# slobodaapl/nvit

Measured on AMD Instinct MI355X. Metric: images/sec (train step) nViT-B/16 224px, higher is better.
Workload: dtype bf16; 1 GPU; nViT-base 224px patches 8/16 T=784 C=768 L=12 H=12, full train step (fwd+bwd+clip+AdamW+renorm), synthetic images, formula weights; per_gpu_batch=128, global_batch=128, parallelism=dp1

## Files before the change

### nvit_amd/csrc/attn_mfma.hip

```cpp
#include <type_traits>

#include "common.h"

namespace {

constexpr int D = 64;
constexpr int ROWB = D * 2;
constexpr int TKV = 64;
constexpr int TILE_BYTES = TKV * ROWB;
constexpr float LOG2E = 1.4426950408889634f;

typedef __attribute__((address_space(3))) s16x4* lds_s16x4_ptr;

__device__ __forceinline__ float fast_exp2(float x) { return __builtin_amdgcn_exp2f(x); }

__device__ __forceinline__ int swz_off(int row, int chunk) { return row * ROWB + ((chunk ^ (row & 7)) << 4); }

__device__ __forceinline__ f32x4 mfma16(const uint4& a, const uint4& b, f32x4 c) {
  return __builtin_amdgcn_mfma_f32_16x16x32_bf16(__builtin_bit_cast(bf16x8, a), __builtin_bit_cast(bf16x8, b), c, 0, 0, 0);
}

__device__ __forceinline__ uint4 tr_frag(const char* tile, int row0, int col0, int l15, int lg) {
  const int q = l15 >> 2, p = l15 & 3;
  const int r0 = row0 + 4 * lg + q, r1 = r0 + 16;
// ... 21 lines not shown

__device__ __forceinline__ void store_tile32x64(const f32x4 (&g)[4][2], char* scr, bf16* dst, size_t ld, int nvalid,
                                                int lane) {
  const int l15 = lane & 15, lg = lane >> 4;
#pragma unroll
  for (int f = 0; f < 2; ++f)
#pragma unroll
    for (int df = 0; df < 4; ++df)
      *reinterpret_cast<uint2*>(scr + swz_off(16 * f + l15, 2 * df + (lg >> 1)) + 8 * (lg & 1)) = pack4(g[df][f]);
  __builtin_amdgcn_wave_barrier();
#pragma unroll
  for (int pass = 0; pass < 4; ++pass) {
    const int row = pass * 8 + (lane >> 3), chunk = lane & 7;
    const uint4 v = *reinterpret_cast<const uint4*>(scr + swz_off(row, chunk));
    if (row < nvalid) *reinterpret_cast<uint4*>(dst + (size_t)row * ld + chunk * 8) = v;
  }
}

__device__ __forceinline__ void glds16s(const void* sbase, unsigned voff, unsigned lds_off) {
  unsigned keep;
  const unsigned m = (unsigned)__builtin_amdgcn_readfirstlane((int)lds_off);
  const unsigned long long ub = (unsigned long long)(uintptr_t)sbase;
  const unsigned long long sb = (unsigned long long)(unsigned)__builtin_amdgcn_readfirstlane((int)(unsigned)ub) |
                                ((unsigned long long)(unsigned)__builtin_amdgcn_readfirstlane((int)(unsigned)(ub >> 32)) << 32);
  asm volatile(
      "s_mov_b32 %0, m0\n\ts_mov_b32 m0, %3\n\ts_nop 0\n\tglobal_load_lds_dwordx4 %1, %2\n\ts_mov_b32 m0, %0"
      : "=&s"(keep)
      : "v"(voff), "s"(sb), "s"(m)
      : "memory");
}
__device__ __forceinline__ void glds16s_pair(const void* sbase, unsigned voff0, unsigned voff1, unsigned lds_off) {
  unsigned keep;
  const unsigned m = (unsigned)__builtin_amdgcn_readfirstlane((int)lds_off);
  const unsigned long long ub = (unsigned long long)(uintptr_t)sbase;
  const unsigned long long sb = (unsigned long long)(unsigned)__builtin_amdgcn_readfirstlane((int)(unsigned)ub) |
                                ((unsigned long long)(unsigned)__builtin_amdgcn_readfirstlane((int)(unsigned)(ub >> 32)) << 32);
  asm volatile(
      "s_mov_b32 %0, m0\n\t"
      "s_mov_b32 m0, %4\n\ts_nop 0\n\tglobal_load_lds_dwordx4 %1, %3\n\t"
      "s_add_u32 m0, %4, 0x1000\n\ts_nop 0\n\tglobal_load_lds_dwordx4 %2, %3\n\t"
      "s_mov_b32 m0, %0"
      : "=&s"(keep)
      : "v"(voff0), "v"(voff1), "s"(sb), "s"(m)
      : "memory", "scc");
}
constexpr int TILE_DMA = 2;
__device__ __forceinline__ unsigned tile_voff(int i, unsigned ld_bytes, int lane, int wid) {
  const int r8 = lane >> 3, chunk = (lane & 7) ^ r8;
  return (unsigned)((i * 4 + wid) * 8 + r8) * ld_bytes + (unsigned)chunk * 16u;
}
__device__ __forceinline__ void tile_dma(const bf16* src, unsigned ld_bytes, int row_base, int nrows, unsigned tile_off,
                                         int lane, int wid, const unsigned (&voff)[TILE_DMA]) {
  const char* sb = reinterpret_cast<const char*>(src) + (size_t)row_base * ld_bytes;
  if (row_base + TKV <= nrows) {
    static_assert(TILE_DMA == 2, "glds16s_pair issues the tile's two pieces");
    glds16s_pair(sb, voff[0], voff[1], tile_off + wid * 1024);
  } else {
    const int r8 = lane >> 3, chunk = (lane & 7) ^ r8;
#pragma unroll
    for (int i = 0; i < TILE_DMA; ++i) {
      const int grp = i * 4 + wid;
      int row = grp * 8 + r8;
      row = row_base + row < nrows ? row : nrows - 1 - row_base;
      glds16s(sb, (unsigned)row * ld_bytes + (unsigned)chunk * 16u, tile_off + grp * 1024);
    }
  }
}
__device__ __forceinline__ void settle(uint4& v) { asm volatile("" : "+v"(v.x), "+v"(v.y), "+v"(v.z), "+v"(v.w)); }
__device__ __forceinline__ void settle(float& v) { asm volatile("" : "+v"(v)); }

__device__ __forceinline__ unsigned lds_addr(const void* p) {
  return (unsigned)(uintptr_t)((__attribute__((address_space(3))) void*)p);
}

__device__ __forceinline__ int work_index() {
  const int nwg = gridDim.x, bid = blockIdx.x;
  const int xcd = bid & 7, q = nwg >> 3, r = nwg & 7;
  return (xcd < r ? xcd * (q + 1) : r * (q + 1) + (xcd - r) * q) + (bid >> 3);
}
__device__ __forceinline__ void work_of(int ntile, int& bh, int& tile) {
  const int w = work_index();
  bh = w / ntile;
  tile = w - bh * ntile;
}

constexpr float BOUND_MAX = 60.0f;

__global__ __launch_bounds__(256, 3) void attn_fwd_mfma_kernel(const bf16* __restrict__ qh, const bf16* __restrict__ kh,
                                                             const bf16* __restrict__ vh, float scale, float qpre,
                                                             const float* __restrict__ sqk, float c_q,
                                                             bf16* __restrict__ o, float* __restrict__ lse, int H,
                                                             int Tq, int Tk) {
  __shared__ __attribute__((aligned(16))) char lds[3][2][TILE_BYTES];
  const int tid = threadIdx.x, lane = tid & 63, wid = tid >> 6;
  const int l15 = lane & 15, lg = lane >> 4;
  int bh, tile_;
  work_of((Tq + 127) / 128, bh, tile_);
  const int b = bh / H, h = bh % H;
  const int q0 = tile_ * 128 + wid * 32;
  const bf16* kbase = kh + (size_t)bh * Tk * D;
  const bf16* vbase = vh + (size_t)bh * Tk * D;
  const float c2t = scale * LOG2E;
  const float c2 = c2t / qpre;
  const bool unit = __builtin_amdgcn_readfirstlane(fabsf(c2 - 1.0f) < 1e-6f ? 1 : 0) != 0;

  uint4 qf[2][2];
  f32x4 oacc[4][2];
#pragma unroll
  for (int i = 0; i < 4; ++i)
#pragma unroll
    for (int f = 0; f < 2; ++f) oacc[i][f] = (f32x4){0.f, 0.f, 0.f, 0.f};
  float m_[2] = {-INFINITY, -INFINITY}, l_[2] = {0.f, 0.f};
  float tb = INFINITY;
  if (sqk) {
    float sm = fabsf(sqk[h * D + lane] * c_q);
#pragma unroll
    for (int off = 32; off > 0; off >>= 1) sm = fmaxf(sm, __shfl_xor(sm, off, 64));
    tb = c2t * sm * sm;
  }
  const bool fast = __builtin_amdgcn_readfirstlane(tb <= BOUND_MAX ? 1 : 0) != 0;
  f32x4 lacc[2] = {(f32x4){0.f, 0.f, 0.f, 0.f}, (f32x4){0.f, 0.f, 0.f, 0.f}};
  const uint4 ones = make_uint4(0x3F803F80u, 0x3F803F80u, 0x3F803F80u, 0x3F803F80u);

  const int nt = (Tk + TKV - 1) / TKV;
  const unsigned ring = lds_addr(&lds[0][0][0]);
  const unsigned voff[TILE_DMA] = {tile_voff(0, ROWB, lane, wid), tile_voff(1, ROWB, lane, wid)};
  tile_dma(kbase, ROWB, 0, Tk, ring, lane, wid, voff);
  tile_dma(vbase, ROWB, 0, Tk, ring + TILE_BYTES, lane, wid, voff);
  if (nt > 1) {
    tile_dma(kbase, ROWB, TKV, Tk, ring + 2 * TILE_BYTES, lane, wid, voff);
    tile_dma(vbase, ROWB, TKV, Tk, ring + 3 * TILE_BYTES, lane, wid, voff);
  }
#pragma unroll
  for (int f = 0; f < 2; ++f) {
    int q = q0 + 16 * f + l15;
    q = q < Tq ? q : Tq - 1;
#pragma unroll
    for (int ks = 0; ks < 2; ++ks)
      qf[f][ks] = *reinterpret_cast<const uint4*>(qh + ((size_t)bh * Tq + q) * D + ks * 32 + lg * 8);
  }
#pragma unroll
  for (int f = 0; f < 2; ++f)
#pragma unroll
    for (int ks = 0; ks < 2; ++ks) settle(qf[f][ks]);
  asm volatile("s_waitcnt vmcnt(0)" ::: "memory");
  __syncthreads();
  int cur = 0;
  const bool wave_active = q0 < Tq;
  f32x4 ntb = {-tb, -tb, -tb, -tb};
  asm volatile("" : "+v"(ntb));
  auto tile_body = [&](const int t, auto masked_, auto fast_, auto unit_) {
    constexpr bool MASKED = decltype(masked_)::value;
    constexpr bool FAST = decltype(fast_)::value;
    constexpr bool UNIT = decltype(unit_)::value;
    if (t + 2 < nt) {
      const int sl = cur == 0 ? 2 : cur - 1;
      tile_dma(kbase, ROWB, (t + 2) * TKV, Tk, ring + (2 * sl) * TILE_BYTES, lane, wid, voff);
      tile_dma(vbase, ROWB, (t + 2) * TKV, Tk, ring + (2 * sl + 1) * TILE_BYTES, lane, wid, voff);
    }
    if (wave_active && FAST) {
      const char* kt = &lds[cur][0][0];
      const char* vt = &lds[cur][1][0];
      const int nvalid = MASKED ? Tk - t * TKV : TKV;
      const int nkf = MASKED ? (nvalid + 15) >> 4 : 4, ns2 = MASKED ? (nvalid + 31) >> 5 : 2;
      uint4 pf[2][2];
#pragma unroll
      for (int s2 = 0; s2 < 2; ++s2) {
        f32x4 p_[2][2];
#pragma unroll
        for (int kk = 0; kk < 2; ++kk) {
          const int kf = 2 * s2 + kk;
          if (!MASKED || kf < nkf) {
            const uint4 a0 = row_frag(kt, kf * 16, 0, l15, lg), a1 = row_frag(kt, kf * 16, 1, l15, lg);
#pragma unroll
            for (int f = 0; f < 2; ++f) {
              f32x4 z = UNIT ? ntb : (f32x4){0.f, 0.f, 0.f, 0.f};
              z = mfma16(a0, qf[f][0], z);
              z = mfma16(a1, qf[f][1], z);
#pragma unroll
              for (int r = 0; r < 4; ++r) {
                float p = UNIT ? fast_exp2(z[r]) : fast_exp2(z[r] * c2 - tb);
                if (MASKED && kf * 16 + lg * 4 + r >= nvalid) p = 0.f;
                p_[kk][f][r] = p;
              }
            }
          } else {
            p_[kk][0] = (f32x4){0.f, 0.f, 0.f, 0.f};
            p_[kk][1] = p_[kk][0];
          }
        }
#pragma unroll
        for (int f = 0; f < 2; ++f) pf[s2][f] = pack8(p_[0][f], p_[1][f]);
      }
#pragma unroll
      for (int s2 = 0; s2 < 2; ++s2)
        if (!MASKED || s2 < ns2) {
#pragma unroll
          for (int f = 0; f < 2; ++f) lacc[f] = mfma16(ones, pf[s2][f], lacc[f]);
#pragma unroll
          for (int df = 0; df < 4; ++df) {
            const uint4 va = tr_frag(vt, s2 * 32, df * 16, l15, lg);
#pragma unroll
            for (int f = 0; f < 2; ++f) oacc[df][f] = mfma16(va, pf[s2][f], oacc[df][f]);
          }
        }
// ... 131 lines not shown
  uint2 xr[2][4];
  float rn[2];
  f32x4 s[4];
};
__device__ __forceinline__ void qk_bwd_epilogue_loads(QkEpiLoads& L, const bf16* xh_bh, const QkFuse& fu, int row0, int T, int H,
                                                      int b, int h, int lane) {
  if (!fu.sqk) return;
  const int l15 = lane & 15, lg = lane >> 4;
#pragma unroll
  for (int f = 0; f < 2; ++f) {
    const int row = row0 + 16 * f + l15;
    const int rc = row < T ? row : T - 1;
#pragma unroll
    for (int df = 0; df < 4; ++df)
      L.xr[f][df] = *reinterpret_cast<const uint2*>(xh_bh + (size_t)rc * 64 + df * 16 + 4 * lg);
    L.rn[f] = fu.rn[((size_t)b * T + rc) * H + h];
  }
#pragma unroll
  for (int df = 0; df < 4; ++df) L.s[df] = *reinterpret_cast<const f32x4*>(fu.sqk + h * 64 + df * 16 + 4 * lg);
}

template <int CTRL>
__device__ __forceinline__ float dpp_add(float v) {
  const int o = __builtin_amdgcn_update_dpp(0, __builtin_bit_cast(int, v), CTRL, 0xF, 0xF, true);
  return v + __builtin_bit_cast(float, o);
}

__device__ __forceinline__ void qk_bwd_epilogue(f32x4 (&g)[4][2], const QkEpiLoads& L, const QkFuse& fu, int row0, int T,
                                                int H, int b, int h, int lane, int wid, char* lds0, int tile,
                                                int ntile, int t256, bool item_valid = true) {
  if (!fu.sqk) {
    if (row0 < T)
      store_tile32x64(g, lds0 + wid * 4096, fu.out + ((size_t)b * T + row0) * fu.ld + h * 64, (size_t)fu.ld, T - row0, lane);
    return;
  }
  const int l15 = lane & 15, lg = lane >> 4;
  float* red = reinterpret_cast<float*>(lds0 + 16384);
  f32x4 s[4], sinv[4], ds[4];
#pragma unroll
  for (int df = 0; df < 4; ++df) {
    s[df] = L.s[df] * fu.c_q;
    ds[df] = (f32x4){0.f, 0.f, 0.f, 0.f};
#pragma unroll
    for (int e = 0; e < 4; ++e) sinv[df][e] = s[df][e] != 0.f ? __builtin_amdgcn_rcpf(s[df][e]) * fu.xs : 0.f;
  }
  f32x4 outv[4][2];
#pragma unroll
  for (int f = 0; f < 2; ++f) {
    const bool valid = row0 + 16 * f + l15 < T;
    f32x4 n[4], sg[4];
    float dot = 0.f;
#pragma unroll
    for (int df = 0; df < 4; ++df) {
      const bf16x4 xb = __builtin_bit_cast(bf16x4, L.xr[f][df]);
      n[df] = (f32x4){(float)xb[0], (float)xb[1], (float)xb[2], (float)xb[3]} * sinv[df];
      if (valid) ds[df] += g[df][f] * n[df];
      sg[df] = g[df][f] * s[df];
      dot += sg[df][0] * n[df][0] + sg[df][1] * n[df][1] + sg[df][2] * n[df][2] + sg[df][3] * n[df][3];
    }
    dot += __shfl_xor(dot, 16, 64);
    dot += __shfl_xor(dot, 32, 64);
#pragma unroll
    for (int df = 0; df < 4; ++df) outv[df][f] = (sg[df] - n[df] * dot) * L.rn[f];
  }
  if (row0 < T)
    store_tile32x64(outv, lds0 + wid * 4096, fu.out + ((size_t)b * T + row0) * fu.ld + h * 64, (size_t)fu.ld, T - row0, lane);
  float pick = 0.f;
#pragma unroll
  for (int df = 0; df < 4; ++df)
#pragma unroll
    for (int e = 0; e < 4; ++e) {
      float v = ds[df][e];
      v = dpp_add<0xB1>(v);
      v = dpp_add<0x4E>(v);
      v = dpp_add<0x141>(v);
      v = dpp_add<0x140>(v);
      pick = l15 == df * 4 + e ? v : pick;
    }
  red[wid * 64 + (l15 >> 2) * 16 + 4 * lg + (l15 & 3)] = pick;
  __syncthreads();
  if (t256 < 64 && item_valid) {
    const float t = red[t256] + red[64 + t256] + red[128 + t256] + red[192 + t256];
    fu.part[((size_t)b * ntile + tile) * (H * 64) + h * 64 + t256] = t;
  }
}

template <bool FUSE>
__global__ __launch_bounds__(256, 3) void attn_bwd_dq_mfma_kernel(const bf16* __restrict__ dout, const bf16* __restrict__ qh,
                                                                const bf16* __restrict__ kh, const bf16* __restrict__ vh,
                                                                const float* __restrict__ lse,
                                                                const bf16* __restrict__ og, float* __restrict__ delta,
                                                                float scale, float qpre, bf16* __restrict__ dqh, int H,
                                                                int Tq, int Tk, QkFuse fu) {
  __shared__ __attribute__((aligned(16))) char lds[3][2][TILE_BYTES];
  const int tid = threadIdx.x, lane = tid & 63, wid = tid >> 6;
  const int l15 = lane & 15, lg = lane >> 4;
  int bh, tile_;
  work_of((Tq + 127) / 128, bh, tile_);
  const int b = bh / H, h = bh % H;
  const int q0 = tile_ * 128 + wid * 32;
  const bf16* kbase = kh + (size_t)bh * Tk * D;
  const bf16* vbase = vh + (size_t)bh * Tk * D;
  const float c2 = scale * LOG2E / qpre;
  const bool unit = __builtin_amdgcn_readfirstlane(fabsf(c2 - 1.0f) < 1e-6f ? 1 : 0) != 0;

  uint4 qf[2][2], gf[2][2];
  float lse2[2], dl[2];
  const int nt = (Tk + TKV - 1) / TKV;
  const unsigned ring = lds_addr(&lds[0][0][0]);
  const unsigned voff[TILE_DMA] = {tile_voff(0, ROWB, lane, wid), tile_voff(1, ROWB, lane, wid)};
  tile_dma(kbase, ROWB, 0, Tk, ring, lane, wid, voff);
  tile_dma(vbase, ROWB, 0, Tk, ring + TILE_BYTES, lane, wid, voff);
  if (nt > 1) {
    tile_dma(kbase, ROWB, TKV, Tk, ring + 2 * TILE_BYTES, lane, wid, voff);
    tile_dma(vbase, ROWB, TKV, Tk, ring + 3 * TILE_BYTES, lane, wid, voff);
  }
#pragma unroll
  for (int f = 0; f < 2; ++f) {
    const int qu = q0 + 16 * f + l15;
    const int q = qu < Tq ? qu : Tq - 1;
    lse2[f] = lse[(size_t)bh * Tq + q] * LOG2E;
#pragma unroll
    for (int ks = 0; ks < 2; ++ks) {
      qf[f][ks] = *reinterpret_cast<const uint4*>(qh + ((size_t)bh * Tq + q) * D + ks * 32 + lg * 8);
      gf[f][ks] = *reinterpret_cast<const uint4*>(dout + ((size_t)b * Tq + q) * (H * D) + h * D + ks * 32 + lg * 8);
    }
    if (og) {
      float part = 0.f;
#pragma unroll
      for (int ks = 0; ks < 2; ++ks) {
        const uint4 of = *reinterpret_cast<const uint4*>(og + ((size_t)b * Tq + q) * (H * D) + h * D + ks * 32 + lg * 8);
        const bf16x8 a = __builtin_bit_cast(bf16x8, gf[f][ks]), c = __builtin_bit_cast(bf16x8, of);
#pragma unroll
        for (int e = 0; e < 8; ++e) part += (float)a[e] * (float)c[e];
      }
      part += __shfl_xor(part, 16, 64);
      part += __shfl_xor(part, 32, 64);
      dl[f] = part;
      if (lg == 0 && qu < Tq) {
        delta[(size_t)bh * Tq + qu] = -part;
        delta[((size_t)(gridDim.x / ((Tq + 127) / 128)) + bh) * Tq + qu] = -lse2[f];
      }
    } else {
      dl[f] = -delta[(size_t)bh * Tq + q];
    }
  }
  f32x4 dq[4][2];
#pragma unroll
  for (int i = 0; i < 4; ++i)
#pragma unroll
    for (int f = 0; f < 2; ++f) dq[i][f] = (f32x4){0.f, 0.f, 0.f, 0.f};
#pragma unroll
  for (int f = 0; f < 2; ++f) {
    settle(lse2[f]);
    settle(dl[f]);
#pragma unroll
    for (int ks = 0; ks < 2; ++ks) {
      settle(qf[f][ks]);
      settle(gf[f][ks]);
    }
  }
  asm volatile("s_waitcnt vmcnt(0)" ::: "memory");
  __syncthreads();
  f32x4 ndl[2], nls[2];
#pragma unroll
  for (int f = 0; f < 2; ++f) {
    ndl[f] = (f32x4){-dl[f], -dl[f], -dl[f], -dl[f]};
    nls[f] = (f32x4){-lse2[f], -lse2[f], -lse2[f], -lse2[f]};
    asm volatile("" : "+v"(ndl[f]));
    asm volatile("" : "+v"(nls[f]));
  }
  int cur = 0;
  const bool wave_active = q0 < Tq;
  auto tile_body = [&](const int t, auto masked_, auto unit_) {
    constexpr bool MASKED = decltype(masked_)::value;
    constexpr bool UNIT = decltype(unit_)::value;
    if (t + 2 < nt) {
      const int sl = cur == 0 ? 2 : cur - 1;
      tile_dma(kbase, ROWB, (t + 2) * TKV, Tk, ring + (2 * sl) * TILE_BYTES, lane, wid, voff);
      tile_dma(vbase, ROWB, (t + 2) * TKV, Tk, ring + (2 * sl + 1) * TILE_BYTES, lane, wid, voff);
    }
    if (wave_active) {
      const char* kt = &lds[cur][0][0];
      const char* vt = &lds[cur][1][0];
      const int kbase_i = t * TKV;
      const int nvalid = MASKED ? Tk - kbase_i : TKV;
      const int nkf = MASKED ? (nvalid + 15) >> 4 : 4, ns2 = MASKED ? (nvalid + 31) >> 5 : 2;
// ... 7 lines not shown
            const int kf = 2 * s2 + kk;
            if (!MASKED || kf < nkf) {
              const uint4 a0 = row_frag(kt, kf * 16, 0, l15, lg), a1 = row_frag(kt, kf * 16, 1, l15, lg);
              const uint4 v0 = row_frag(vt, kf * 16, 0, l15, lg), v1 = row_frag(vt, kf * 16, 1, l15, lg);
#pragma unroll
              for (int f = 0; f < 2; ++f) {
                f32x4 z = UNIT ? nls[f] : (f32x4){0.f, 0.f, 0.f, 0.f};
                z = mfma16(a0, qf[f][0], z);
                z = mfma16(a1, qf[f][1], z);
                f32x4 w = mfma16(v0, gf[f][0], ndl[f]);
                w = mfma16(v1, gf[f][1], w);
#pragma unroll
                for (int r = 0; r < 4; ++r) {
                  const bool valid = !MASKED || (kf * 16 + lg * 4 + r) < nvalid;
                  const float p = valid ? (UNIT ? fast_exp2(z[r]) : fast_exp2(z[r] * c2 - lse2[f])) : 0.f;
                  ds_[kk][f][r] = p * w[r];
                }
              }
            } else {
              ds_[kk][0] = (f32x4){0.f, 0.f, 0.f, 0.f};
              ds_[kk][1] = ds_[kk][0];
            }
          }
#pragma unroll
          for (int f = 0; f < 2; ++f) dsf[s2][f] = pack8(ds_[0][f], ds_[1][f]);
        }
      }
#pragma unroll
      for (int df = 0; df < 4; ++df)
#pragma unroll
        for (int s2 = 0; s2 < 2; ++s2)
          if (!MASKED || s2 < ns2) {
            const uint4 ka = tr_frag(kt, s2 * 32, df * 16, l15, lg);
#pragma unroll
            for (int f = 0; f < 2; ++f) dq[df][f] = mfma16(ka, dsf[s2][f], dq[df][f]);
          }
    }
    if (t + 2 < nt)
      asm volatile("s_waitcnt vmcnt(%0)" ::"n"(4) : "memory");
    else
      asm volatile("s_waitcnt vmcnt(0)" ::: "memory");
    __syncthreads();
    cur = cur == 2 ? 0 : cur + 1;
  };
#define NVIT_RUN_TILES(UNIT_)                                                          \
  {                                                                                    \
    for (int t = 0; t + 1 < nt; ++t) tile_body(t, std::false_type{}, UNIT_{});         \
    if (Tk % TKV)                                                                      \
      tile_body(nt - 1, std::true_type{}, UNIT_{});                                    \
    else                                                                               \
      tile_body(nt - 1, std::false_type{}, UNIT_{});                                   \
  }
  if (unit)
    NVIT_RUN_TILES(std::true_type)
  else
    NVIT_RUN_TILES(std::false_type)
#undef NVIT_RUN_TILES
#pragma unroll
  for (int i = 0; i < 4; ++i)
#pragma unroll
    for (int f = 0; f < 2; ++f) dq[i][f] = dq[i][f] * scale;
  if constexpr (FUSE) {
    QkEpiLoads el;
    qk_bwd_epilogue_loads(el, qh + (size_t)bh * Tq * D, fu, q0, Tq, H, b, h, lane);
    qk_bwd_epilogue(dq, el, fu, q0, Tq, H, b, h, lane, wid, &lds[0][0][0], tile_, (Tq + 127) / 128, (int)threadIdx.x);
  } else {
    if (wave_active)
      store_tile32x64(dq, &lds[0][0][0] + wid * 4096, dqh + ((size_t)bh * Tq + q0) * D, (size_t)D, Tq - q0, lane);
  }
}

__device__ __forceinline__ void glds4a(const void* gsrc, unsigned lds_off) {
  unsigned keep;
  const unsigned m = (unsigned)__builtin_amdgcn_readfirstlane((int)lds_off);
  asm volatile(
      "s_mov_b32 %0, m0\n\ts_mov_b32 m0, %2\n\ts_nop 0\n\tglobal_load_lds_dword %1, off\n\ts_mov_b32 m0, %0"
      : "=&s"(keep)
      : "v"(gsrc), "s"(m)
      : "memory");
}
constexpr int DKV_SLOT = 2 * TILE_BYTES + 512;
constexpr int DKV_DMA = 2 * TILE_DMA + 2;
constexpr int DKV_WAVES = 2;

template <bool FUSE>
__global__ __launch_bounds__(256, DKV_WAVES) void attn_bwd_dkv_mfma_kernel(const bf16* __restrict__ dout, const bf16* __restrict__ qh,
                                                                 const bf16* __restrict__ kh, const bf16* __restrict__ vh,
                                                                 const float* __restrict__ lse,
                                                                 const float* __restrict__ delta, float scale,
                                                                 float qpre, bf16* __restrict__ dkh,
                                                                 bf16* __restrict__ dvh, int H, int Tq, int Tk,
                                                                 QkFuse fu) {
  __shared__ __attribute__((aligned(16))) char lds[3 * DKV_SLOT];
  const int tid = threadIdx.x, lane = tid & 63;
  const int wid = __builtin_amdgcn_readfirstlane(tid >> 6);
  const int l15 = lane & 15, lg = lane >> 4;
  int bh, tile_;
  work_of((Tk + 127) / 128, bh, tile_);
  const int b = bh / H, h = bh % H;
  const int k0 = tile_ * 128 + wid * 32;
  const bf16* qbase = qh + (size_t)bh * Tq * D;
  const bf16* gbase = dout + (size_t)b * Tq * (H * D) + h * D;
  const float* dbase = delta + (size_t)bh * Tq;
  const float* lbase = delta + ((size_t)(gridDim.x / ((Tk + 127) / 128)) + bh) * Tq;
  const float c2 = scale * LOG2E / qpre;
  const bool unit = __builtin_amdgcn_readfirstlane(fabsf(c2 - 1.0f) < 1e-6f ? 1 : 0) != 0;
  const int nt = (Tq + TKV - 1) / TKV;
  const unsigned ring = lds_addr(&lds[0]);

  const unsigned ldg_bytes = (unsigned)(H * D * 2);
  const unsigned voff_q[TILE_DMA] = {tile_voff(0, ROWB, lane, wid), tile_voff(1, ROWB, lane, wid)};
  const unsigned voff_g[TILE_DMA] = {tile_voff(0, ldg_bytes, lane, wid), tile_voff(1, ldg_bytes, lane, wid)};
  auto tile_issue = [&](int t, int slot) {
    const unsigned so = ring + (unsigned)slot * DKV_SLOT;
    tile_dma(qbase, ROWB, t * TKV, Tq, so, lane, wid, voff_q);
    tile_dma(gbase, ldg_bytes, t * TKV, Tq, so + TILE_BYTES, lane, wid, voff_g);
    int q = t * TKV + lane;
    q = q < Tq ? q : Tq - 1;
    glds4a(lbase + q, so + 2 * TILE_BYTES);
    glds4a(dbase + q, so + 2 * TILE_BYTES + 256);
  };
  tile_issue(0, 0);
  if (nt > 1) tile_issue(1, 1);

  uint4 kf_[2][2], vf_[2][2];
#pragma unroll
  for (int f = 0; f < 2; ++f) {
    int k = k0 + 16 * f + l15;
    k = k < Tk ? k : Tk - 1;
#pragma unroll
    for (int ks = 0; ks < 2; ++ks) {
      kf_[f][ks] = *reinterpret_cast<const uint4*>(kh + ((size_t)bh * Tk + k) * D + ks * 32 + lg * 8);
      vf_[f][ks] = *reinterpret_cast<const uint4*>(vh + ((size_t)bh * Tk + k) * D + ks * 32 + lg * 8);
    }
  }
#pragma unroll
  for (int f = 0; f < 2; ++f)
#pragma unroll
    for (int ks = 0; ks < 2; ++ks) {
      settle(kf_[f][ks]);
      settle(vf_[f][ks]);
    }
  asm volatile("s_waitcnt vmcnt(0)" ::: "memory");
  __syncthreads();

  f32x4 dk[4][2], dv[4][2];
#pragma unroll
  for (int i = 0; i < 4; ++i)
#pragma unroll
    for (int f = 0; f < 2; ++f) {
      dk[i][f] = (f32x4){0.f, 0.f, 0.f, 0.f};
      dv[i][f] = (f32x4){0.f, 0.f, 0.f, 0.f};
    }
  const bool wave_active = k0 < Tk;
  int cur = 0;
  auto tile_body = [&](const int t, auto masked_, auto unit_) {
    constexpr bool MASKED = decltype(masked_)::value;
    constexpr bool UNIT = decltype(unit_)::value;
    if (t + 2 < nt) tile_issue(t + 2, cur == 0 ? 2 : cur - 1);
    if (wave_active) {
      const char* qt = &lds[cur * DKV_SLOT];
      const char* gt = qt + TILE_BYTES;
      const float* st = reinterpret_cast<const float*>(qt + 2 * TILE_BYTES);
      const int nvalid = MASKED ? Tq - t * TKV : TKV;
      const int nqf = MASKED ? (nvalid + 15) >> 4 : 4, ns2 = MASKED ? (nvalid + 31) >> 5 : 2;
      if constexpr (!MASKED) {
#pragma unroll
        for (int s2 = 0; s2 < 2; ++s2) {
          uint4 a[2][2], gg[2][2], ga[4], qa[4];
          f32x4 nl[2], nd[2];
#pragma unroll
          for (int qq = 0; qq < 2; ++qq) {
            const int qfi = 2 * s2 + qq;
            a[qq][0] = row_frag(qt, qfi * 16, 0, l15, lg), a[qq][1] = row_frag(qt, qfi * 16, 1, l15, lg);
            gg[qq][0] = row_frag(gt, qfi * 16, 0, l15, lg), gg[qq][1] = row_frag(gt, qfi * 16, 1, l15, lg);
            nl[qq] = *reinterpret_cast<const f32x4*>(st + qfi * 16 + 4 * lg);
            nd[qq] = *reinterpret_cast<const f32x4*>(st + 64 + qfi * 16 + 4 * lg);
          }
#pragma unroll
          for (int df = 0; df < 4; ++df) {
            ga[df] = tr_frag(gt, s2 * 32, df * 16, l15, lg);
            qa[df] = tr_frag(qt, s2 * 32, df * 16, l15, lg);
          }
// ... 85 lines not shown
#pragma unroll
        for (int df = 0; df < 4; ++df) {
          const uint4 ga = tr_frag(gt, s2 * 32, df * 16, l15, lg);
          const uint4 qa = tr_frag(qt, s2 * 32, df * 16, l15, lg);
#pragma unroll
          for (int f = 0; f < 2; ++f) {
            dv[df][f] = mfma16(ga, pb[f], dv[df][f]);
            dk[df][f] = mfma16(qa, sb[f], dk[df][f]);
          }
        }
      }
    }
    if (t + 2 < nt)
      asm volatile("s_waitcnt vmcnt(%0)" ::"n"(DKV_DMA) : "memory");
    else
      asm volatile("s_waitcnt vmcnt(0)" ::: "memory");
    __syncthreads();
    cur = cur == 2 ? 0 : cur + 1;
  };
#define NVIT_RUN_TILES(UNIT_)                                                          \
  {                                                                                    \
    for (int t = 0; t + 1 < nt; ++t) tile_body(t, std::false_type{}, UNIT_{});         \
    if (Tq % TKV)                                                                      \
      tile_body(nt - 1, std::true_type{}, UNIT_{});                                    \
    else                                                                               \
      tile_body(nt - 1, std::false_type{}, UNIT_{});                                   \
  }
  if (unit)
    NVIT_RUN_TILES(std::true_type)
  else
    NVIT_RUN_TILES(std::false_type)
#undef NVIT_RUN_TILES
  const float dks = scale / qpre;
#pragma unroll
  for (int i = 0; i < 4; ++i)
#pragma unroll
    for (int f = 0; f < 2; ++f) dk[i][f] = dk[i][f] * dks;
  char* scr = &lds[0] + wid * 4096;
  if constexpr (FUSE) {
    if (wave_active)
      store_tile32x64(dv, scr, fu.out_v + ((size_t)b * Tk + k0) * fu.ld + h * 64, (size_t)fu.ld, Tk - k0, lane);
    __builtin_amdgcn_wave_barrier();
    QkEpiLoads el;
    qk_bwd_epilogue_loads(el, kh + (size_t)bh * Tk * D, fu, k0, Tk, H, b, h, lane);
    qk_bwd_epilogue(dk, el, fu, k0, Tk, H, b, h, lane, wid, &lds[0], tile_, (Tk + 127) / 128, (int)threadIdx.x);
  } else {
    if (wave_active) {
      store_tile32x64(dk, scr, dkh + ((size_t)bh * Tk + k0) * D, (size_t)D, Tk - k0, lane);
      __builtin_amdgcn_wave_barrier();
      store_tile32x64(dv, scr, dvh + ((size_t)bh * Tk + k0) * D, (size_t)D, Tk - k0, lane);
    }
  }
}


__device__ __forceinline__ unsigned uni32(unsigned x) { return (unsigned)__builtin_amdgcn_readfirstlane((int)x); }
__device__ __forceinline__ unsigned long long uni64(const void* p) {
  const unsigned long long u = (unsigned long long)(uintptr_t)p;
  return (unsigned long long)uni32((unsigned)u) | ((unsigned long long)uni32((unsigned)(u >> 32)) << 32);
}

#include "attn_dkv32_asm.inc"

template <bool FUSE>
__global__ __launch_bounds__(256, 2) void attn_bwd_dkv_asm32_kernel(const bf16* __restrict__ dout, const bf16* __restrict__ qh,
                                                                  const bf16* __restrict__ kh, const bf16* __restrict__ vh,
                                                                  const float* __restrict__ delta, float scale, float qpre,
                                                                  bf16* __restrict__ dkh, bf16* __restrict__ dvh, int H,
                                                                  int Tq, int Tk, const float* fu_rn, const float* fu_sqk,
                                                                  float fu_cq, bf16* fu_out, bf16* fu_outv, int fu_ld,
                                                                  float* fu_part, float fu_xs) {
  __shared__ __attribute__((aligned(16))) char lds[4 * DKV_SLOT];
  static_assert(4 * DKV_SLOT >= 4 * 16384, "the hand-over area must fit the ring");
  const int tid = threadIdx.x;
  int lane = tid & 63;
  const int wid = (int)uni32((unsigned)(tid >> 6));
  const int l15 = lane & 15, lg = lane >> 4;
  int bh, tile_;
  const int ntile = (Tk + 127) / 128;
  work_of(ntile, bh, tile_);
  const int b = bh / H, h = bh % H;
  const int k0 = tile_ * 128 + wid * 32;
  const int BH = gridDim.x / ntile;
  const int nt = (Tq + TKV - 1) / TKV;
  const int nvalid_last = Tq - (nt - 1) * TKV;
  const unsigned ldg = (unsigned)(H * D * 2);
  const int r8 = lane >> 3, chunk = (lane & 7) ^ r8;
  const unsigned voff_q0 = tile_voff(0, ROWB, lane, wid), voff_g0 = tile_voff(0, ldg, lane, wid);
  unsigned rows_last = 0;
#pragma unroll
  for (int i = 0; i < 2; ++i) {
    int row = (i * 4 + wid) * 8 + r8;
    row = row < nvalid_last ? row : nvalid_last - 1;
    rows_last |= (unsigned)row << (8 * i);
  }
  unsigned kvoff[2];
#pragma unroll
  for (int f = 0; f < 2; ++f) {
    int k = k0 + 16 * f + l15;
    k = k < Tk ? k : Tk - 1;
    kvoff[f] = (unsigned)(k * D + lg * 8) * 2u;
  }
  const unsigned a0 = (unsigned)swz_off(l15, lg), a1 = (unsigned)swz_off(l15, 4 + lg);
  unsigned tro[4];
#pragma unroll
  for (int df = 0; df < 4; ++df)
    tro[df] = (unsigned)(swz_off(4 * lg + (l15 >> 2), 2 * df + ((l15 & 3) >> 1)) + ((l15 & 1) << 3));
  const unsigned ring = lds_addr(&lds[0]);
  const unsigned dump = ring + (unsigned)wid * 16384u + (unsigned)lane * 16u;
  const unsigned long long s_q = uni64(qh + (size_t)bh * Tq * D);
  const unsigned long long s_g = uni64(dout + (size_t)b * Tq * (H * D) + h * D);
  const unsigned long long s_l = uni64(delta + ((size_t)BH + bh) * Tq);
  const unsigned long long s_d = uni64(delta + (size_t)bh * Tq);
  const unsigned long long s_k = uni64(kh + (size_t)bh * Tk * D);
  const unsigned long long s_v = uni64(vh + (size_t)bh * Tk * D);
  const unsigned s_nt = uni32((unsigned)nt), s_ldg = uni32(ldg), s_ring = uni32(ring), s_nvl = uni32((unsigned)nvalid_last);
  const unsigned s_act = uni32(k0 < Tk ? 1u : 0u), s_wofs = uni32((unsigned)wid * 1024u);
  asm volatile(NVIT_ATTN_DKV32_ASM_BODY
               :
               : "s"(s_q), "s"(s_g), "s"(s_l), "s"(s_d), "s"(s_k), "s"(s_v), "s"(s_nt), "s"(s_ldg), "s"(s_ring), "s"(s_nvl),
                 "s"(s_act), "s"(s_wofs), "v"(voff_q0), "v"(voff_g0), "v"(rows_last), "v"((unsigned)chunk * 16u),
                 "v"((unsigned)lane * 4u), "v"(kvoff[0]), "v"(kvoff[1]), "v"(a0), "v"(a1), "v"((unsigned)(lg * 16)), "v"(tro[0]),
                 "v"(tro[1]), "v"(tro[2]), "v"(tro[3]),
                 "v"(dump)
               : NVIT_ATTN_DKV32_ASM_CLOBBERS);
  int tid2 = threadIdx.x;
  asm volatile("" : "+v"(tid2));
  lane = tid2 & 63;
  const QkFuse fu{fu_rn, fu_sqk, fu_out, fu_outv, fu_part, fu_cq, fu_xs, fu_ld};
  const bool wave_active = k0 < Tk;
  QkEpiLoads el;
  if constexpr (FUSE) qk_bwd_epilogue_loads(el, kh + (size_t)bh * Tk * D, fu, k0, Tk, H, b, h, lane);
  f32x4 dk[4][2], dv[4][2];
  if (wave_active) {
    const char* mine = &lds[0] + wid * 16384 + lane * 16;
#pragma unroll
    for (int df = 0; df < 4; ++df)
#pragma unroll
      for (int f = 0; f < 2; ++f) {
        dk[df][f] = *reinterpret_cast<const f32x4*>(mine + (df * 2 + f) * 1024);
        dv[df][f] = *reinterpret_cast<const f32x4*>(mine + (8 + df * 2 + f) * 1024);
      }
  }
  __syncthreads();
  const float dks = scale / qpre;
#pragma unroll
  for (int i = 0; i < 4; ++i)
#pragma unroll
    for (int f = 0; f < 2; ++f) dk[i][f] = dk[i][f] * dks;
  char* scr = &lds[0] + wid * 4096;
  if constexpr (FUSE) {
    if (wave_active)
      store_tile32x64(dv, scr, fu.out_v + ((size_t)b * Tk + k0) * fu.ld + h * 64, (size_t)fu.ld, Tk - k0, lane);
    __builtin_amdgcn_wave_barrier();
    qk_bwd_epilogue(dk, el, fu, k0, Tk, H, b, h, lane, wid, &lds[0], tile_, ntile, (int)threadIdx.x);
  } else {
    if (wave_active) {
      store_tile32x64(dk, scr, dkh + ((size_t)bh * Tk + k0) * D, (size_t)D, Tk - k0, lane);
      __builtin_amdgcn_wave_barrier();
      store_tile32x64(dv, scr, dvh + ((size_t)bh * Tk + k0) * D, (size_t)D, Tk - k0, lane);
    }
  }
}

int g_attn_dkv_asm = 1;
int dkv_asm_mode(float scale, float qpre) {
// ... 739 lines not shown
```

Before: 1281 images/sec.

## Split KV loop across waves for 16-row tail tiles in attention kernels

Adds dedicated tail paths to the forward, dQ and dK/dV attention kernels for the last tile when it holds 16 or fewer rows. In the original layout only one wave of the block does useful work on such a tile, yet it walks the whole KV/Q sequence. In the new path each of the four waves handles a 16-row slice of every 64-row tile, and the partial accumulators are summed through LDS at the end. This shortens those straggler blocks, at the cost of extra code, an LDS reduction and raised wave priority.

```diff
diff --git a/nvit_amd/csrc/attn_mfma.hip b/nvit_amd/csrc/attn_mfma.hip
--- a/nvit_amd/csrc/attn_mfma.hip
+++ b/nvit_amd/csrc/attn_mfma.hip
@@ -127,6 +127,93 @@
   const int w = work_index();
   bh = w / ntile;
   tile = w - bh * ntile;
+}
+
+__device__ __forceinline__ bool tail_block(int T, int tile) { return T - tile * 128 <= 16; }
+
+template <int N>
+__device__ __forceinline__ void tail_sum(f32x4 (&acc)[N], char* lds0, int w, int lane) {
+  f32x4* all = reinterpret_cast<f32x4*>(lds0);
+#pragma unroll
+  for (int i = 0; i < N; ++i) all[(w * N + i) * 64 + lane] = acc[i];
+  __syncthreads();
+  if (w == 0) {
+#pragma unroll
+    for (int i = 0; i < N; ++i)
+      acc[i] = ((all[i * 64 + lane] + all[(N + i) * 64 + lane]) + all[(2 * N + i) * 64 + lane]) + all[(3 * N + i) * 64 + lane];
+  }
+  __syncthreads();
+}
+
+__device__ __forceinline__ void attn_fwd_tail(const bf16* __restrict__ qh, const bf16* kbase, const bf16* vbase, float c2,
+                                              float tb, bf16* __restrict__ o, float* __restrict__ lse, char* lds0, int b,
+                                              int h, int bh, int H, int Tq, int Tk, int qb, int lane, int w) {
+  __builtin_amdgcn_s_setprio(3);
+  const int l15 = lane & 15, lg = lane >> 4;
+  const int nt = (Tk + TKV - 1) / TKV;
+  const unsigned ring = lds_addr(lds0);
+  const unsigned voff[TILE_DMA] = {tile_voff(0, ROWB, lane, w), tile_voff(1, ROWB, lane, w)};
+  auto tile_issue = [&](int t, int slot) {
+    tile_dma(kbase, ROWB, t * TKV, Tk, ring + (2 * slot) * TILE_BYTES, lane, w, voff);
+    tile_dma(vbase, ROWB, t * TKV, Tk, ring + (2 * slot + 1) * TILE_BYTES, lane, w, voff);
+  };
+  tile_issue(0, 0);
+  if (nt > 1) tile_issue(1, 1);
+  uint4 qf[2];
+  {
+    int q = qb + l15;
+    q = q < Tq ? q : Tq - 1;
+#pragma unroll
+    for (int ks = 0; ks < 2; ++ks) qf[ks] = *reinterpret_cast<const uint4*>(qh + ((size_t)bh * Tq + q) * D + ks * 32 + lg * 8);
+  }
+  settle(qf[0]);
+  settle(qf[1]);
+  asm volatile("s_waitcnt vmcnt(0)" ::: "memory");
+  __syncthreads();
+  const f32x4 zero = {0.f, 0.f, 0.f, 0.f};
+  f32x4 acc[5] = {zero, zero, zero, zero, zero};
+  const uint4 ones = make_uint4(0x3F803F80u, 0x3F803F80u, 0x3F803F80u, 0x3F803F80u);
+  const int s2 = w >> 1;
+  const bool hi = (w & 1) != 0;
+  int cur = 0;
+  for (int t = 0; t < nt; ++t) {
+    if (t + 2 < nt) tile_issue(t + 2, cur == 0 ? 2 : cur - 1);
+    const int nvalid = Tk - t * TKV < TKV ? Tk - t * TKV : TKV;
+    if (w * 16 < nvalid) {
+      const char* kt = lds0 + (2 * cur) * TILE_BYTES;
+      const char* vt = kt + TILE_BYTES;
+      const uint4 a0 = row_frag(kt, w * 16, 0, l15, lg), a1 = row_frag(kt, w * 16, 1, l15, lg);
+      f32x4 z = mfma16(a0, qf[0], zero);
+      z = mfma16(a1, qf[1], z);
+      f32x4 p;
+#pragma unroll
+      for (int r = 0; r < 4; ++r) p[r] = w * 16 + lg * 4 + r < nvalid ? fast_exp2(z[r] * c2 - tb) : 0.f;
+      const uint4 pf = hi ? pack8(zero, p) : pack8(p, zero);
+      acc[4] = mfma16(ones, pf, acc[4]);
+#pragma unroll
+      for (int df = 0; df < 4; ++df) acc[df] = mfma16(tr_frag(vt, s2 * 32, df * 16, l15, lg), pf, acc[df]);
+    }
+    if (t + 2 < nt)
+      asm volatile("s_waitcnt vmcnt(%0)" ::"n"(4) : "memory");
+    else
+      asm volatile("s_waitcnt vmcnt(0)" ::: "memory");
+    __syncthreads();
+    cur = cur == 2 ? 0 : cur + 1;
+  }
+  tail_sum(acc, lds0, w, lane);
+  if (w == 0) {
+    const float l = acc[4][0];
+    const float inv = 1.0f / l;
+    f32x4 g[4][2];
+#pragma unroll
+    for (int df = 0; df < 4; ++df) {
+      g[df][0] = acc[df] * inv;
+      g[df][1] = zero;
+    }
+    const int q = qb + l15;
+    if (q < Tq && lg == 0) lse[(size_t)bh * Tq + q] = (tb + log2f(l)) * (1.0f / LOG2E);
+    store_tile32x64(g, lds0, o + ((size_t)b * Tq + qb) * (H * D) + h * D, (size_t)H * D, Tq - qb, lane);
+  }
 }
 
 constexpr float BOUND_MAX = 60.0f;
@@ -166,6 +253,11 @@
   const bool fast = __builtin_amdgcn_readfirstlane(tb <= BOUND_MAX ? 1 : 0) != 0;
   f32x4 lacc[2] = {(f32x4){0.f, 0.f, 0.f, 0.f}, (f32x4){0.f, 0.f, 0.f, 0.f}};
   const uint4 ones = make_uint4(0x3F803F80u, 0x3F803F80u, 0x3F803F80u, 0x3F803F80u);
+  if (fast && tail_block(Tq, tile_)) {
+    attn_fwd_tail(qh, kbase, vbase, c2, tb, o, lse, &lds[0][0][0], b, h, bh, H, Tq, Tk, tile_ * 128, lane,
+                  __builtin_amdgcn_readfirstlane(wid));
+    return;
+  }
 
   const int nt = (Tk + TKV - 1) / TKV;
   const unsigned ring = lds_addr(&lds[0][0][0]);
@@ -463,6 +555,113 @@
   if (t256 < 64 && item_valid) {
     const float t = red[t256] + red[64 + t256] + red[128 + t256] + red[192 + t256];
     fu.part[((size_t)b * ntile + tile) * (H * 64) + h * 64 + t256] = t;
+  }
+}
+
+template <bool FUSE>
+__device__ __forceinline__ void attn_bwd_dq_tail(const bf16* __restrict__ dout, const bf16* __restrict__ qh, const bf16* kbase,
+                                                 const bf16* vbase, const float* __restrict__ lse,
+                                                 const bf16* __restrict__ og, float* __restrict__ delta, float scale, float c2,
+                                                 bf16* __restrict__ dqh, int H, int Tq, int Tk, const QkFuse& fu, char* lds0,
+                                                 int b, int h, int bh, int tile, int ntile, int BH, int lane, int w) {
+  __builtin_amdgcn_s_setprio(3);
+  const int l15 = lane & 15, lg = lane >> 4;
+  const int qb = tile * 128;
+  const int nt = (Tk + TKV - 1) / TKV;
+  const unsigned ring = lds_addr(lds0);
+  const unsigned voff[TILE_DMA] = {tile_voff(0, ROWB, lane, w), tile_voff(1, ROWB, lane, w)};
+  auto tile_issue = [&](int t, int slot) {
+    tile_dma(kbase, ROWB, t * TKV, Tk, ring + (2 * slot) * TILE_BYTES, lane, w, voff);
+    tile_dma(vbase, ROWB, t * TKV, Tk, ring + (2 * slot + 1) * TILE_BYTES, lane, w, voff);
+  };
+  tile_issue(0, 0);
+  if (nt > 1) tile_issue(1, 1);
+  uint4 qf[2], gf[2];
+  float lse2, dl;
+  {
+    const int qu = qb + l15;
+    const int q = qu < Tq ? qu : Tq - 1;
+    lse2 = lse[(size_t)bh * Tq + q] * LOG2E;
+#pragma unroll
+    for (int ks = 0; ks < 2; ++ks) {
+      qf[ks] = *reinterpret_cast<const uint4*>(qh + ((size_t)bh * Tq + q) * D + ks * 32 + lg * 8);
+      gf[ks] = *reinterpret_cast<const uint4*>(dout + ((size_t)b * Tq + q) * (H * D) + h * D + ks * 32 + lg * 8);
+    }
+    if (og) {
+      float part = 0.f;
+#pragma unroll
+      for (int ks = 0; ks < 2; ++ks) {
+        const uint4 of = *reinterpret_cast<const uint4*>(og + ((size_t)b * Tq + q) * (H * D) + h * D + ks * 32 + lg * 8);
+        const bf16x8 a = __builtin_bit_cast(bf16x8, gf[ks]), c = __builtin_bit_cast(bf16x8, of);
+#pragma unroll
+        for (int e = 0; e < 8; ++e) part += (float)a[e] * (float)c[e];
+      }
+      part += __shfl_xor(part, 16, 64);
+      part += __shfl_xor(part, 32, 64);
+      dl = part;
+      if (w == 0 && lg == 0 && qu < Tq) {
+        delta[(size_t)bh * Tq + qu] = -part;
+        delta[((size_t)BH + bh) * Tq + qu] = -lse2;
+      }
+    } else {
+      dl = -delta[(size_t)bh * Tq + q];
+    }
+  }
+  settle(lse2);
+  settle(dl);
+#pragma unroll
+  for (int ks = 0; ks < 2; ++ks) {
+    settle(qf[ks]);
+    settle(gf[ks]);
+  }
+  asm volatile("s_waitcnt vmcnt(0)" ::: "memory");
+  __syncthreads();
+  const f32x4 zero = {0.f, 0.f, 0.f, 0.f};
+  const f32x4 ndl = {-dl, -dl, -dl, -dl};
+  f32x4 dq[4] = {zero, zero, zero, zero};
+  const int s2 = w >> 1;
+  const bool hi = (w & 1) != 0;
+  int cur = 0;
+  for (int t = 0; t < nt; ++t) {
+    if (t + 2 < nt) tile_issue(t + 2, cur == 0 ? 2 : cur - 1);
+    const int nvalid = Tk - t * TKV < TKV ? Tk - t * TKV : TKV;
+    if (w * 16 < nvalid) {
+      const char* kt = lds0 + (2 * cur) * TILE_BYTES;
+      const char* vt = kt + TILE_BYTES;
+      const uint4 a0 = row_frag(kt, w * 16, 0, l15, lg), a1 = row_frag(kt, w * 16, 1, l15, lg);
+      const uint4 v0 = row_frag(vt, w * 16, 0, l15, lg), v1 = row_frag(vt, w * 16, 1, l15, lg);
+      f32x4 z = mfma16(a0, qf[0], zero);
+      z = mfma16(a1, qf[1], z);
+      f32x4 dp = mfma16(v0, gf[0], ndl);
+      dp = mfma16(v1, gf[1], dp);
+      f32x4 ds;
+#pragma unroll
+      for (int r = 0; r < 4; ++r) ds[r] = w * 16 + lg * 4 + r < nvalid ? fast_exp2(z[r] * c2 - lse2) * dp[r] : 0.f;
+      const uint4 dsf = hi ? pack8(zero, ds) : pack8(ds, zero);
+#pragma unroll
+      for (int df = 0; df < 4; ++df) dq[df] = mfma16(tr_frag(kt, s2 * 32, df * 16, l15, lg), dsf, dq[df]);
+    }
+    if (t + 2 < nt)
+      asm volatile("s_waitcnt vmcnt(%0)" ::"n"(4) : "memory");
+    else
+      asm volatile("s_waitcnt vmcnt(0)" ::: "memory");
+    __syncthreads();
+    cur = cur == 2 ? 0 : cur + 1;
+  }
+  tail_sum(dq, lds0, w, lane);
+  f32x4 g[4][2];
+#pragma unroll
+  for (int df = 0; df < 4; ++df) {
+    g[df][0] = w == 0 ? dq[df] * scale : zero;
+    g[df][1] = zero;
+  }
+  const int q0 = qb + w * 32;
+  if constexpr (FUSE) {
+    QkEpiLoads el;
+    qk_bwd_epilogue_loads(el, qh + (size_t)bh * Tq * D, fu, q0, Tq, H, b, h, lane);
+    qk_bwd_epilogue(g, el, fu, q0, Tq, H, b, h, lane, w, lds0, tile, ntile, (int)threadIdx.x);
+  } else {
+    if (w == 0) store_tile32x64(g, lds0, dqh + ((size_t)bh * Tq + qb) * D, (size_t)D, Tq - qb, lane);
   }
 }
 
@@ -484,6 +683,12 @@
   const bf16* vbase = vh + (size_t)bh * Tk * D;
   const float c2 = scale * LOG2E / qpre;
   const bool unit = __builtin_amdgcn_readfirstlane(fabsf(c2 - 1.0f) < 1e-6f ? 1 : 0) != 0;
+  if (tail_block(Tq, tile_)) {
+    const int ntile = (Tq + 127) / 128;
+    attn_bwd_dq_tail<FUSE>(dout, qh, kbase, vbase, lse, og, delta, scale, c2, dqh, H, Tq, Tk, fu, &lds[0][0][0], b, h, bh,
+                           tile_, ntile, (int)gridDim.x / ntile, lane, __builtin_amdgcn_readfirstlane(wid));
+    return;
+  }
 
   uint4 qf[2][2], gf[2][2];
   float lse2[2], dl[2];
@@ -657,6 +862,122 @@
 constexpr int DKV_SLOT = 2 * TILE_BYTES + 512;
 constexpr int DKV_DMA = 2 * TILE_DMA + 2;
 constexpr int DKV_WAVES = 2;
+
+template <bool FUSE>
+__device__ __forceinline__ void attn_bwd_dkv_tail(const bf16* __restrict__ dout, const bf16* __restrict__ qh,
+                                                  const bf16* __restrict__ kh, const bf16* __restrict__ vh,
+                                                  const float* __restrict__ delta, float scale, float qpre,
+                                                  bf16* __restrict__ dkh, bf16* __restrict__ dvh, int H, int Tq, int Tk,
+                                                  const QkFuse& fu, char* lds0, int b, int h, int bh, int tile, int ntile,
+                                                  int BH, int lane, int w) {
+  __builtin_amdgcn_s_setprio(3);
+  const int l15 = lane & 15, lg = lane >> 4;
+  const int kb = tile * 128;
+  const bf16* qbase = qh + (size_t)bh * Tq * D;
+  const bf16* gbase = dout + (size_t)b * Tq * (H * D) + h * D;
+  const float* dbase = delta + (size_t)bh * Tq;
+  const float* lbase = delta + ((size_t)BH + bh) * Tq;
+  const float c2 = scale * LOG2E / qpre;
+  const int nt = (Tq + TKV - 1) / TKV;
+  const unsigned ring = lds_addr(lds0);
+  const unsigned ldg_bytes = (unsigned)(H * D * 2);
+  const unsigned voff_q[TILE_DMA] = {tile_voff(0, ROWB, lane, w), tile_voff(1, ROWB, lane, w)};
+  const unsigned voff_g[TILE_DMA] = {tile_voff(0, ldg_bytes, lane, w), tile_voff(1, ldg_bytes, lane, w)};
+  auto tile_issue = [&](int t, int slot) {
+    const unsigned so = ring + (unsigned)slot * DKV_SLOT;
+    tile_dma(qbase, ROWB, t * TKV, Tq, so, lane, w, voff_q);
+    tile_dma(gbase, ldg_bytes, t * TKV, Tq, so + TILE_BYTES, lane, w, voff_g);
+    int q = t * TKV + lane;
+    q = q < Tq ? q : Tq - 1;
+    glds4a(lbase + q, so + 2 * TILE_BYTES);
+    glds4a(dbase + q, so + 2 * TILE_BYTES + 256);
+  };
+  tile_issue(0, 0);
+  if (nt > 1) tile_issue(1, 1);
+  uint4 kf_[2], vf_[2];
+  {
+    int k = kb + l15;
+    k = k < Tk ? k : Tk - 1;
+#pragma unroll
+    for (int ks = 0; ks < 2; ++ks) {
+      kf_[ks] = *reinterpret_cast<const uint4*>(kh + ((size_t)bh * Tk + k) * D + ks * 32 + lg * 8);
+      vf_[ks] = *reinterpret_cast<const uint4*>(vh + ((size_t)bh * Tk + k) * D + ks * 32 + lg * 8);
+    }
+  }
+#pragma unroll
+  for (int ks = 0; ks < 2; ++ks) {
+    settle(kf_[ks]);
+    settle(vf_[ks]);
+  }
+  asm volatile("s_waitcnt vmcnt(0)" ::: "memory");
+  __syncthreads();
+  const f32x4 zero = {0.f, 0.f, 0.f, 0.f};
+  f32x4 acc[8] = {zero, zero, zero, zero, zero, zero, zero, zero};
+  const int s2 = w >> 1;
+  const bool hi = (w & 1) != 0;
+  int cur = 0;
+  for (int t = 0; t < nt; ++t) {
+    if (t + 2 < nt) tile_issue(t + 2, cur == 0 ? 2 : cur - 1);
+    const int nvalid = Tq - t * TKV < TKV ? Tq - t * TKV : TKV;
+    if (w * 16 < nvalid) {
+      const char* qt = lds0 + cur * DKV_SLOT;
+      const char* gt = qt + TILE_BYTES;
+      const float* st = reinterpret_cast<const float*>(qt + 2 * TILE_BYTES);
+      const uint4 a0 = row_frag(qt, w * 16, 0, l15, lg), a1 = row_frag(qt, w * 16, 1, l15, lg);
+      const uint4 g0 = row_frag(gt, w * 16, 0, l15, lg), g1 = row_frag(gt, w * 16, 1, l15, lg);
+      const f32x4 nl4 = *reinterpret_cast<const f32x4*>(st + w * 16 + 4 * lg);
+      const f32x4 nd4 = *reinterpret_cast<const f32x4*>(st + 64 + w * 16 + 4 * lg);
+      f32x4 z = mfma16(a0, kf_[0], zero);
+      z = mfma16(a1, kf_[1], z);
+      f32x4 dp = mfma16(g0, vf_[0], nd4);
+      dp = mfma16(g1, vf_[1], dp);
+      f32x4 p, dsv;
+#pragma unroll
+      for (int r = 0; r < 4; ++r) {
+        p[r] = w * 16 + lg * 4 + r < nvalid ? fast_exp2(z[r] * c2 + nl4[r]) : 0.f;
+        dsv[r] = p[r] * dp[r];
+      }
+      const uint2 ph = pack4(p), sh = pack4(dsv);
+      const uint4 pb = hi ? make_uint4(0u, 0u, ph.x, ph.y) : make_uint4(ph.x, ph.y, 0u, 0u);
+      const uint4 sb = hi ? make_uint4(0u, 0u, sh.x, sh.y) : make_uint4(sh.x, sh.y, 0u, 0u);
+#pragma unroll
+      for (int df = 0; df < 4; ++df) {
+        acc[4 + df] = mfma16(tr_frag(gt, s2 * 32, df * 16, l15, lg), pb, acc[4 + df]);
+        acc[df] = mfma16(tr_frag(qt, s2 * 32, df * 16, l15, lg), sb, acc[df]);
+      }
+    }
+    if (t + 2 < nt)
+      asm volatile("s_waitcnt vmcnt(%0)" ::"n"(DKV_DMA) : "memory");
+    else
+      asm volatile("s_waitcnt vmcnt(0)" ::: "memory");
+    __syncthreads();
+    cur = cur == 2 ? 0 : cur + 1;
+  }
+  tail_sum(acc, lds0, w, lane);
+  const float dks = scale / qpre;
+  f32x4 dk[4][2], dv[4][2];
+#pragma unroll
+  for (int df = 0; df < 4; ++df) {
+    dk[df][0] = w == 0 ? acc[df] * dks : zero;
+    dv[df][0] = w == 0 ? acc[4 + df] : zero;
+    dk[df][1] = zero;
+    dv[df][1] = zero;
+  }
+  const int k0 = kb + w * 32;
+  if constexpr (FUSE) {
+    if (w == 0) store_tile32x64(dv, lds0, fu.out_v + ((size_t)b * Tk + kb) * fu.ld + h * 64, (size_t)fu.ld, Tk - kb, lane);
+    __builtin_amdgcn_wave_barrier();
+    QkEpiLoads el;
+    qk_bwd_epilogue_loads(el, kh + (size_t)bh * Tk * D, fu, k0, Tk, H, b, h, lane);
+    qk_bwd_epilogue(dk, el, fu, k0, Tk, H, b, h, lane, w, lds0, tile, ntile, (int)threadIdx.x);
+  } else {
+    if (w == 0) {
+      store_tile32x64(dk, lds0, dkh + ((size_t)bh * Tk + kb) * D, (size_t)D, Tk - kb, lane);
+      __builtin_amdgcn_wave_barrier();
+      store_tile32x64(dv, lds0, dvh + ((size_t)bh * Tk + kb) * D, (size_t)D, Tk - kb, lane);
+    }
+  }
+}
 
 template <bool FUSE>
 __global__ __launch_bounds__(256, DKV_WAVES) void attn_bwd_dkv_mfma_kernel(const bf16* __restrict__ dout, const bf16* __restrict__ qh,
@@ -674,6 +995,12 @@
   work_of((Tk + 127) / 128, bh, tile_);
   const int b = bh / H, h = bh % H;
   const int k0 = tile_ * 128 + wid * 32;
+  if (tail_block(Tk, tile_)) {
+    const int ntile = (Tk + 127) / 128;
+    attn_bwd_dkv_tail<FUSE>(dout, qh, kh, vh, delta, scale, qpre, dkh, dvh, H, Tq, Tk, fu, &lds[0], b, h, bh, tile_, ntile,
+                            (int)gridDim.x / ntile, lane, wid);
+    return;
+  }
   const bf16* qbase = qh + (size_t)bh * Tq * D;
   const bf16* gbase = dout + (size_t)b * Tq * (H * D) + h * D;
   const float* dbase = delta + (size_t)bh * Tq;
@@ -925,6 +1252,14 @@
   const int b = bh / H, h = bh % H;
   const int k0 = tile_ * 128 + wid * 32;
   const int BH = gridDim.x / ntile;
+  if (tail_block(Tk, tile_)) {
+    int tid1 = threadIdx.x;
+    asm volatile("" : "+v"(tid1));
+    const QkFuse fu{fu_rn, fu_sqk, fu_out, fu_outv, fu_part, fu_cq, fu_xs, fu_ld};
+    attn_bwd_dkv_tail<FUSE>(dout, qh, kh, vh, delta, scale, qpre, dkh, dvh, H, Tq, Tk, fu, &lds[0], b, h, bh, tile_, ntile, BH,
+                            tid1 & 63, (int)uni32((unsigned)(tid1 >> 6)));
+    return;
+  }
   const int nt = (Tq + TKV - 1) / TKV;
   const int nvalid_last = Tq - (nt - 1) * TKV;
   const unsigned ldg = (unsigned)(H * D * 2);
```

New measurement: 1284 images/sec, median of 3. Within noise of the previous version (+0.2%).
